# LemonATsu/UNet-PhaseGen

Measured on NVIDIA B200. Metric: audio_seconds_per_second_mag_to_phase_to_wave, higher is better.
Workload: dtype f16x3/f16x2/f16-fp32acc (two-product fp16 on d1,u2; single fp16 product = TF32 operand rounding on u1)

## Files before the change

unet-phasegen_b200/csrc/conv_tc.cu:

```cuda
#include "tc_ptx.cuh"
#include "conv_plan.h"

namespace pg {

struct ConvTcParams {
    ConvPlan plan;
    float* y;
    float4* stats;
    int n_a_slots;
    int b_slot_bytes;
    int n_terms;
    int f16;
    int base_offset_mode;
    int a_mn;
    int epi_mode;
    const float* gamma; const float* beta; float eps;
    ActDst dst0, dst1;
    float2* ss_out;
    const int* clip_rows;
};

constexpr int kThreads = 192;
constexpr int kATileBytes = 128 * 128;
constexpr int kMaxASlots = 8;

struct TileCoord { int co_tile, phase, b0, nt; };

__device__ __forceinline__ int n_bundles(const ConvPlan& p) { return (p.B + p.nb - 1) / p.nb; }
__device__ __forceinline__ int n_co_slabs(const ConvPlan& p) { return p.pair ? p.n_cotiles / 2 : p.n_cotiles; }
__device__ __forceinline__ int tile_OS(const ConvPlan& p) { return p.whole_clip ? 1 : p.OS; }
__device__ __forceinline__ int tile_NT(const ConvPlan& p) { return p.whole_clip ? 1 : p.n_ntiles; }
__device__ __forceinline__ int total_tiles(const ConvPlan& p) { return n_co_slabs(p) * tile_OS(p) * n_bundles(p) * tile_NT(p); }
__device__ __forceinline__ TileCoord decode_tile(const ConvPlan& p, int tile) {
    TileCoord c;
    const int OSx = tile_OS(p), NTx = tile_NT(p);
    const int nbg = n_bundles(p), G = p.clip_group, n_slabs = n_co_slabs(p) * OSx;
    const int tiles_full = n_slabs * G * NTx;
    const int g = tile / tiles_full, r = tile % tiles_full;
    int Gg = nbg - g * G; if (Gg > G) Gg = G;
    const int per_slab = Gg * NTx;
    const int slab = r / per_slab, r2 = r % per_slab;
    c.co_tile = slab / OSx; c.phase = slab % OSx;
    c.b0 = (g * G + r2 / NTx) * p.nb; c.nt = r2 % NTx;
    return c;
}

template <bool PAIR, bool RAGGED>
__global__ void __launch_bounds__(kThreads, 1)
conv_tc_kernel(const __grid_constant__ CUtensorMap map_w_hi, const __grid_constant__ CUtensorMap map_w_lo,
               const __grid_constant__ CUtensorMap map_x_hi, const __grid_constant__ CUtensorMap map_x_lo,
               const __grid_constant__ ConvTcParams prm) {
    extern __shared__ __align__(1024) uint8_t smem_raw[];
    const ConvPlan& pl = prm.plan;
    uint8_t* smem = reinterpret_cast<uint8_t*>((reinterpret_cast<uintptr_t>(smem_raw) + 1023) & ~uintptr_t(1023));
    const int nA = prm.n_a_slots;
    const int bPlane = prm.b_slot_bytes;
    const int a_planes = prm.n_terms == 3 ? 2 : 1;
    const int b_planes = prm.n_terms >= 2 ? 2 : 1;
    uint8_t* a_base = smem;
    uint8_t* b_base = a_base + (size_t)nA * a_planes * kATileBytes;
    uint64_t* bars = reinterpret_cast<uint64_t*>(b_base + 2 * (size_t)b_planes * bPlane);
    uint64_t* fullA = bars;
    uint64_t* emptyA = bars + kMaxASlots;
    uint64_t* fullB = bars + 2 * kMaxASlots;
    uint64_t* emptyB = fullB + 2;
    uint64_t* accFull = emptyB + 2;
    uint64_t* accEmpty = accFull + 2;
    uint32_t* tmem_slot = reinterpret_cast<uint32_t*>(accEmpty + 2);
    uint32_t* epi_tiles = reinterpret_cast<uint32_t*>(reinterpret_cast<uint8_t*>(bars) + 256);

    const int warp = __shfl_sync(0xffffffffu, (int)(threadIdx.x >> 5), 0), lane = threadIdx.x & 31;
    const int n_tiles = total_tiles(pl);
    const bool w_lo = prm.n_terms == 3, x_lo = prm.n_terms >= 2;

    if (warp == 0 && lane == 0) {
        tma_prefetch_desc(&map_w_hi); tma_prefetch_desc(&map_x_hi);
        if (w_lo) tma_prefetch_desc(&map_w_lo);
        if (x_lo) tma_prefetch_desc(&map_x_lo);
        for (int i = 0; i < nA; ++i) { mbar_init(fullA + i, 1); mbar_init(emptyA + i, 1); }
        for (int i = 0; i < 2; ++i) {
            mbar_init(fullB + i, 1); mbar_init(emptyB + i, 1);
            mbar_init(accFull + i, 1); mbar_init(accEmpty + i, PAIR ? 8 : 4);
        }
        fence_barrier_init();
    }
    if (warp == 1) { if (PAIR) tmem_alloc_pair(tmem_slot, 512); else tmem_alloc(tmem_slot, 512); }
    tc_fence_before();
    if (PAIR) cluster_sync_all(); else __syncthreads();
    tc_fence_after();
    const uint32_t tmem_base = __shfl_sync(0xffffffffu, *tmem_slot, 0);
    const int rank = PAIR ? (int)cluster_ctarank() : 0;
    const int tile0 = PAIR ? (int)(blockIdx.x >> 1) : (int)blockIdx.x;
    const int tile_step = PAIR ? (int)(gridDim.x >> 1) : (int)gridDim.x;
    const int half_n = pl.n_tile >> 1;
    const int nb_grp = pl.nb / pl.mgroups;
    const int nb_cta = (PAIR && pl.merged) ? nb_grp >> 1 : nb_grp;
    const int t_phases = pl.whole_clip ? pl.OS : 1;
    const int t_nts = pl.whole_clip ? pl.n_ntiles : 1;
    const int n_sub = pl.merged ? pl.mgroups : t_nts;

    if (warp == 0) {
        {
            uint32_t b_it = 0;
            int a_slot = 0; uint32_t a_ph = 0;
            const uint32_t grp_bytes = (uint32_t)nb_cta * pl.strip_rows * 128u;
            const uint32_t a_bytes = a_planes * kATileBytes;
            const uint32_t b_bytes = b_planes * (uint32_t)bPlane;
            for (int tile = tile0; tile < n_tiles; tile += tile_step) {
                TileCoord tc = decode_tile(pl, tile);
                if (PAIR) tc.co_tile = tc.co_tile * 2 + rank;
                const int m0 = tc.nt * pl.n_tile + ((PAIR && !pl.merged) ? rank * half_n : 0);
                const int clip0 = tc.b0 + ((PAIR && pl.merged) ? rank * nb_cta : 0);
                for (int ch = 0; ch < pl.n_chunks; ++ch) {
                  for (int ph = tc.phase; ph < tc.phase + t_phases; ++ph) {
                    const int ng = pl.n_groups[ph];
                    for (int g = 0; g < ng; ++g) {
                        const ConvGroup grp = pl.groups[ph][g];
                        {
                            const int s = b_it & 1; const uint32_t bph = (b_it >> 1) & 1;
                            mbar_wait(emptyB + s, bph ^ 1);
                            uint8_t* dst = b_base + (size_t)s * b_planes * bPlane;
                            if (elect_one()) {
                                if (PAIR) { if (rank == 0) mbar_expect_tx(fullB + s, 2 * b_bytes); }
                                else mbar_expect_tx(fullB + s, b_bytes);
                                for (int sub = 0; sub < n_sub; ++sub) {
                                    uint8_t* dg = dst + (size_t)sub * grp_bytes;
                                    const int cg = clip0 + (pl.merged ? sub * nb_grp : 0);
                                    const int r0 = m0 + (pl.merged ? 0 : sub * pl.n_tile) + grp.row0;
                                    if (PAIR) {
                                        tma_load_4d_pair(dg, &map_x_hi, fullB + s, ch * 64, grp.parity, r0, cg);
                                        if (x_lo) tma_load_4d_pair(dg + bPlane, &map_x_lo, fullB + s, ch * 64, grp.parity, r0, cg);
                                    } else {
                                        tma_load_4d(dg, &map_x_hi, fullB + s, ch * 64, grp.parity, r0, cg);
                                        if (x_lo) tma_load_4d(dg + bPlane, &map_x_lo, fullB + s, ch * 64, grp.parity, r0, cg);
                                    }
                                }
                            }
                            __syncwarp();
                            ++b_it;
                        }
                        for (int j = 0; j < grp.n_taps; ++j) {
                            const int w_idx = pl.taps[ph][grp.first_tap + j].w_idx;
                            const int s = a_slot; const uint32_t aph = a_ph;
                            mbar_wait(emptyA + s, aph ^ 1);
                            uint8_t* dst = a_base + (size_t)s * a_planes * kATileBytes;
                            if (elect_one()) {
                                if (!PAIR) mbar_expect_tx(fullA + s, a_bytes);
                                else if (rank == 0) mbar_expect_tx(fullA + s, 2 * a_bytes);
                                auto load_w = [&](uint8_t* d, const CUtensorMap* m, int c0, int c1) {
                                    if (PAIR) tma_load_3d_pair(d, m, fullA + s, c0, c1, w_idx);
                                    else tma_load_3d(d, m, fullA + s, c0, c1, w_idx);
                                };
                                if (prm.a_mn) {
                                    for (int h = 0; h < 2; ++h) {
                                        load_w(dst + h * 8192, &map_w_hi, tc.co_tile * 128 + h * 64, ch * 64);
                                        if (w_lo) load_w(dst + kATileBytes + h * 8192, &map_w_lo, tc.co_tile * 128 + h * 64, ch * 64);
                                    }
                                } else {
                                    load_w(dst, &map_w_hi, ch * 64, tc.co_tile * 128);
                                    if (w_lo) load_w(dst + kATileBytes, &map_w_lo, ch * 64, tc.co_tile * 128);
                                }
                            }
                            __syncwarp();
                            if (++a_slot == nA) { a_slot = 0; a_ph ^= 1; }
                        }
                    }
                  }
                }
            }
        }
    } else if (warp == 1) {
        if (rank == 0) {
            uint32_t b_it = 0, t_it = 0;
            int a_slot = 0; uint32_t a_ph = 0;
            const int n_mma = pl.merged ? nb_grp * pl.strip_rows : pl.n_tile;
            const int n_outer = pl.merged ? 1 : t_nts, n_inner = pl.merged ? pl.mgroups : pl.nb;
            const uint32_t dcol_step = pl.merged ? (uint32_t)n_mma : (uint32_t)(pl.n_tile * t_phases * t_nts);
            const uint32_t idesc = (make_idesc_bf16(n_mma, PAIR ? 256 : 128) & ~(prm.f16 ? ((7u << 7) | (7u << 10)) : 0u)) |
                                   (prm.a_mn ? (1u << 15) : 0u);
            const bool a_mn = prm.a_mn != 0;
            auto mma = [&](uint32_t d, uint32_t da, uint32_t db, uint32_t acc_flag) {
                if (elect_one()) { if (PAIR) umma_words_pair(d, da, db, idesc, acc_flag); else umma_words(d, da, db, idesc, acc_flag); }
            };
            const uint32_t a_step = a_mn ? (2048u >> 4) : (32u >> 4);
            auto commit = [&](uint64_t* bar) {
                if (elect_one()) { if (PAIR) umma_commit_pair(bar); else umma_commit(bar); }
                __syncwarp();
            };
            for (int tile = tile0; tile < n_tiles; tile += tile_step, ++t_it) {
                TileCoord tc = decode_tile(pl, tile);
                const int acc = pl.acc_stages == 2 ? (t_it & 1) : 0;
                const uint32_t acc_ph = pl.acc_stages == 2 ? ((t_it >> 1) & 1) : (t_it & 1);
                mbar_wait_sleep(accEmpty + acc, acc_ph ^ 1, 200);
                tc_fence_after();
                const uint32_t d_tmem = tmem_base + acc * 256;
                const uint32_t strip_bytes = (uint32_t)pl.strip_rows * 128u;
                const uint32_t clip_step = (pl.merged ? (uint32_t)nb_cta * strip_bytes : strip_bytes) >> 4;
                for (int ch = 0; ch < pl.n_chunks; ++ch) {
                  for (int ph = tc.phase; ph < tc.phase + t_phases; ++ph) {
                    const int ng = pl.n_groups[ph];
                    const uint32_t dcol_ph = d_tmem + (uint32_t)((ph - tc.phase) * t_nts * pl.n_tile);
                    for (int g = 0; g < ng; ++g) {
                        const ConvGroup grp = pl.groups[ph][g];
                        const int bs = b_it & 1; const uint32_t bph = (b_it >> 1) & 1;
                        mbar_wait(fullB + bs, bph);
                        tc_fence_after();
                        const uint32_t b_hi = smem_u32(b_base + (size_t)bs * b_planes * bPlane);
                        const uint32_t b_lo = b_hi + bPlane;
                        for (int j = 0; j < grp.n_taps; ++j) {
                            const ConvTap tp = pl.taps[ph][grp.first_tap + j];
                            const int as = a_slot; const uint32_t aph = a_ph;
                            mbar_wait(fullA + as, aph);
                            tc_fence_after();
                            const uint32_t a_hi = smem_u32(a_base + (size_t)as * a_planes * kATileBytes);
                            const uint32_t a_lo = a_hi + kATileBytes;
                            const uint32_t sh = (uint32_t)tp.shift * 128u;
                            const uint32_t acc_first = (ch | g | j) ? 1u : 0u;
                            const uint32_t aw_hi = a_mn ? desc_lo_sw128_mn(a_hi, 8192) : desc_lo_sw128(a_hi);
                            const uint32_t aw_lo = a_mn ? desc_lo_sw128_mn(a_lo, 8192) : desc_lo_sw128(a_lo);
                            uint32_t bw_hi = desc_lo_sw128(b_hi + sh), bw_lo = desc_lo_sw128(b_lo + sh);
                            for (int o = 0; o < n_outer; ++o) {
                                uint32_t dcol = dcol_ph + (uint32_t)o * (uint32_t)pl.n_tile;
                                for (int c = 0; c < n_inner; ++c, bw_hi += clip_step, bw_lo += clip_step, dcol += dcol_step) {
                                    if (w_lo) {
#pragma unroll
                                        for (uint32_t kk = 0; kk < 4; ++kk) {
                                            mma(dcol, aw_lo + kk * a_step, bw_hi + kk * 2, kk == 0 ? acc_first : 1u);
                                            mma(dcol, aw_hi + kk * a_step, bw_lo + kk * 2, 1);
                                            mma(dcol, aw_hi + kk * a_step, bw_hi + kk * 2, 1);
                                        }
                                    } else if (x_lo) {
#pragma unroll
                                        for (uint32_t kk = 0; kk < 4; ++kk) {
                                            mma(dcol, aw_hi + kk * a_step, bw_lo + kk * 2, kk == 0 ? acc_first : 1u);
                                            mma(dcol, aw_hi + kk * a_step, bw_hi + kk * 2, 1);
                                        }
                                    } else {
#pragma unroll
                                        for (uint32_t kk = 0; kk < 4; ++kk) mma(dcol, aw_hi + kk * a_step, bw_hi + kk * 2, kk == 0 ? acc_first : 1u);
                                    }
                                }
                            }
                            commit(emptyA + as);
                            if (++a_slot == nA) { a_slot = 0; a_ph ^= 1; }
                        }
                        commit(emptyB + bs);
                        ++b_it;
                    }
                  }
                }
                commit(accFull + acc);
            }
        }
    } else {
        const int q = warp & 3;
        uint32_t* tile = epi_tiles + q * 512;
        uint32_t t_it = 0;
        const int n_parts = t_phases * t_nts;
        const int col_pitch = pl.merged ? pl.strip_rows : pl.n_tile * n_parts;
        bool bad_range = false;
        auto store_f32 = [&](float* base, size_t off0, size_t row_pitch, const float* v, int nv) {
#pragma unroll
            for (int i = 0; i < 16; ++i) tile[i * 32 + lane] = __float_as_uint(v[i]);
            __syncwarp();
#pragma unroll
            for (int t = 0; t < 4; ++t) {
                const int idx = lane + 32 * t, r = idx >> 3, part = idx & 7;
                if (r < nv) {
                    const uint4 w = *reinterpret_cast<const uint4*>(tile + r * 32 + part * 4);
                    *reinterpret_cast<uint4*>(base + off0 + (size_t)r * row_pitch + part * 4) = w;
                }
            }
            __syncwarp();
        };
        auto store_split = [&](const ActDst& d, size_t off0, size_t row_pitch, const float* v, int nv) {
            const int fmt = fmt_of_dtype(d.dtype);
#pragma unroll
            for (int i = 0; i < 16; ++i) {
                const float a = leaky(v[i], d.slope);
                uint16_t h, l;
                split16(a, fmt, h, l);
                if (fmt == PG_FMT_F16 && i < nv) bad_range |= !f16_fits(a);
                tile[i * 32 + lane] = (uint32_t)h | ((uint32_t)l << 16);
            }
            __syncwarp();
            const bool two = d.dtype == PG_DT_BF16_SPLIT || d.dtype == PG_DT_F16_SPLIT;
#pragma unroll
            for (int t = 0; t < 2; ++t) {
                const int idx = lane + 32 * t, r = idx >> 2, part = idx & 3;
                if (r < nv) {
                    const uint4 w0 = *reinterpret_cast<const uint4*>(tile + r * 32 + part * 8);
                    const uint4 w1 = *reinterpret_cast<const uint4*>(tile + r * 32 + part * 8 + 4);
                    uint4 hv, lv;
                    hv.x = __byte_perm(w0.x, w0.y, 0x5410); hv.y = __byte_perm(w0.z, w0.w, 0x5410);
                    hv.z = __byte_perm(w1.x, w1.y, 0x5410); hv.w = __byte_perm(w1.z, w1.w, 0x5410);
                    lv.x = __byte_perm(w0.x, w0.y, 0x7632); lv.y = __byte_perm(w0.z, w0.w, 0x7632);
                    lv.z = __byte_perm(w1.x, w1.y, 0x7632); lv.w = __byte_perm(w1.z, w1.w, 0x7632);
                    const size_t o = off0 + (size_t)r * row_pitch + part * 8;
                    *reinterpret_cast<uint4*>(static_cast<uint16_t*>(d.hi) + o) = hv;
                    if (two) *reinterpret_cast<uint4*>(static_cast<uint16_t*>(d.lo) + o) = lv;
                }
            }
            __syncwarp();
        };
        for (int tile_i = tile0; tile_i < n_tiles; tile_i += tile_step, ++t_it) {
            TileCoord tc = decode_tile(pl, tile_i);
            if (PAIR) tc.co_tile = tc.co_tile * 2 + rank;
            const int acc = pl.acc_stages == 2 ? (t_it & 1) : 0;
            const uint32_t acc_ph = pl.acc_stages == 2 ? ((t_it >> 1) & 1) : (t_it & 1);
            mbar_wait_sleep(accFull + acc, acc_ph, 1000);
            tc_fence_after();
            const int co_base = tc.co_tile * 128 + q * 32;
            const int co = co_base + lane;
            auto part_geom = [&](int p, int L, int& phase, int& m0, int& n_valid) {
                phase = tc.phase + p / t_nts;
                m0 = (tc.nt + p % t_nts) * pl.n_tile;
                const int l_phase = (L - phase + pl.OS - 1) / pl.OS;
                n_valid = l_phase - m0; if (n_valid > pl.n_tile) n_valid = pl.n_tile; if (n_valid < 0) n_valid = 0;
            };
            for (int c = 0; c < pl.nb; ++c) {
                const int b = tc.b0 + c;
                if (b >= pl.B) break;
                const int L_b = RAGGED ? min(__ldg(prm.clip_rows + b), pl.L_out) : pl.L_out;
                const uint32_t tclip = tmem_base + acc * 256 + c * col_pitch + ((uint32_t)(q * 32) << 16);
                if (prm.epi_mode == PG_EPI_RAW) {
                    for (int p = 0; p < n_parts; ++p) {
                        int phase, m0, n_valid;
                        part_geom(p, L_b, phase, m0, n_valid);
                        const uint32_t taddr = tclip + p * pl.n_tile;
                        float sum = 0.f;
                        for (int c0 = 0; c0 < n_valid; c0 += 16) {
                            float v[16];
                            tmem_ld16(taddr + c0, v);
#pragma unroll
                            for (int i = 0; i < 16; ++i) if (c0 + i < n_valid) sum += v[i];
                        }
                        const float mean = n_valid > 0 ? sum / (float)n_valid : 0.f;
                        float m2 = 0.f;
                        const size_t row_pitch = (size_t)pl.OS * pl.out_ld;
                        for (int c0 = 0; c0 < n_valid; c0 += 16) {
                            float v[16];
                            tmem_ld16(taddr + c0, v);
#pragma unroll
                            for (int i = 0; i < 16; ++i) if (c0 + i < n_valid) { const float d = v[i] - mean; m2 += d * d; }
                            const size_t off0 = ((size_t)b * pl.out_rows + (size_t)(m0 + c0) * pl.OS + phase) * pl.out_ld + co_base;
                            store_f32(prm.y, off0, row_pitch, v, n_valid - c0);
                        }
                        if (prm.stats) {
                            const int P = pl.OS * pl.n_ntiles;
                            const int pi = phase * pl.n_ntiles + m0 / pl.n_tile;
                            prm.stats[((size_t)b * P + pi) * pl.C_out + co] = make_float4((float)n_valid, mean, m2, 0.f);
                        }
                    }
                } else {
                    float sc = 1.f, sh = 0.f;
                    if (prm.epi_mode == PG_EPI_NORM_ACT) {
                        float sum = 0.f; int n_tot = 0;
                        for (int p = 0; p < n_parts; ++p) {
                            int phase, m0, n_valid;
                            part_geom(p, L_b, phase, m0, n_valid);
                            n_tot += n_valid;
                            for (int c0 = 0; c0 < n_valid; c0 += 16) {
                                float v[16];
                                tmem_ld16(tclip + p * pl.n_tile + c0, v);
#pragma unroll
                                for (int i = 0; i < 16; ++i) if (c0 + i < n_valid) sum += v[i];
                            }
                        }
                        const float mean = n_tot > 0 ? sum / (float)n_tot : 0.f;
                        float m2 = 0.f;
                        for (int p = 0; p < n_parts; ++p) {
                            int phase, m0, n_valid;
                            part_geom(p, L_b, phase, m0, n_valid);
                            for (int c0 = 0; c0 < n_valid; c0 += 16) {
                                float v[16];
                                tmem_ld16(tclip + p * pl.n_tile + c0, v);
#pragma unroll
                                for (int i = 0; i < 16; ++i) if (c0 + i < n_valid) { const float d = v[i] - mean; m2 += d * d; }
                            }
                        }
                        const float var = n_tot > 0 ? m2 / (float)n_tot : 0.f;
                        sc = (prm.gamma ? __ldg(prm.gamma + co) : 1.f) * rsqrtf(var + prm.eps);
                        sh = (prm.beta ? __ldg(prm.beta + co) : 0.f) - mean * sc;
                        if (prm.ss_out) prm.ss_out[(size_t)b * pl.C_out + co] = make_float2(sc, sh);
                    }
                    for (int p = 0; p < n_parts; ++p) {
// ... 69 lines not shown
}

void device_limits(int* sm_count, int* max_smem) {
    static int sm_dev[kMaxDevices] = {}, smem_dev[kMaxDevices] = {};
    const int slot = current_device_slot();
    if (!sm_dev[slot]) {
        int dev = 0; cudaGetDevice(&dev);
        cudaDeviceGetAttribute(&sm_dev[slot], cudaDevAttrMultiProcessorCount, dev);
        cudaDeviceGetAttribute(&smem_dev[slot], cudaDevAttrMaxSharedMemoryPerBlockOptin, dev);
    }
    *sm_count = sm_dev[slot]; *max_smem = smem_dev[slot];
}

}

extern "C" int pg_conv_epilogue_supported(const pg_conv_desc* d, int mode) {
    using namespace pg;
    PG_REQUIRE(d, "pg_conv_epilogue_supported: null descriptor");
    if (mode == PG_EPI_RAW) return 1;
    if (mode != PG_EPI_ACT && mode != PG_EPI_NORM_ACT) return 0;
    if (d->precision == PG_PREC_FP32_SIMT || d->C_in % 64 || d->C_out % 128) return 0;
    if (mode == PG_EPI_ACT) return 1;
    pg_conv_desc dd = *d;
    dd.tc_whole_clip = 1;
    ConvPlan pl;
    if (conv_plan_build(&dd, &pl) != PG_OK) return 0;
    return (pl.whole_clip || (pl.OS == 1 && pl.n_ntiles == 1)) ? 1 : 0;
}

static int conv_tc_launch(const pg_conv_desc* d, const uint16_t* x_hi, const uint16_t* x_lo, const uint16_t* w_hi,
                          const uint16_t* w_lo, float* y, float* stats, const pg_conv_epilogue* epi, const int* out_rows,
                          pg_stream stream) {
    using namespace pg;
    const int epi_mode = epi ? epi->mode : PG_EPI_RAW;
    PG_REQUIRE(d && x_hi && w_hi && (y || epi_mode != PG_EPI_RAW), "pg_conv_tc: null pointer");
    PG_REQUIRE(epi_mode == PG_EPI_RAW || epi_mode == PG_EPI_ACT || epi_mode == PG_EPI_NORM_ACT, "pg_conv_tc: bad epilogue mode %d", epi_mode);
    PG_REQUIRE(d->precision >= PG_PREC_BF16X3 && d->precision <= PG_PREC_F16, "pg_conv_tc: precision must be BF16X3, BF16, F16X3, F16X2 or F16");
    const int n_terms = (d->precision == PG_PREC_BF16X3 || d->precision == PG_PREC_F16X3) ? 3 : d->precision == PG_PREC_F16X2 ? 2 : 1;
    const bool three = n_terms == 3;
    PG_REQUIRE(n_terms < 3 || w_lo, "pg_conv_tc: weight lo plane required for the three-product precisions");
    PG_REQUIRE(n_terms < 2 || x_lo, "pg_conv_tc: activation lo plane required for this precision");
    PG_REQUIRE(d->C_in % 64 == 0 && d->C_out % 128 == 0, "pg_conv_tc: needs C_in %% 64 == 0 and C_out %% 128 == 0 (got %d, %d)", d->C_in, d->C_out);
    PG_REQUIRE(d->in_ld % 8 == 0, "pg_conv_tc: input row pitch must be a multiple of 8 elements");
    PG_REQUIRE(d->tc_base_offset_mode == 0, "pg_conv_tc: descriptor base-offset mode 0 is the only supported one (the UMMA swizzle is a "
               "function of the absolute shared-memory address: profiles/r01_tc_probe.log)");
    ConvTcParams prm;
    pg_conv_desc d_local = *d;
    if (const char* e = getenv("PG_TC_PAIR")) d_local.tc_cta_pair = atoi(e);
    d_local.tc_whole_clip = epi_mode == PG_EPI_NORM_ACT ? 1 : 0;
    d = &d_local;
    int rc = conv_plan_build(d, &prm.plan);
    if (rc != PG_OK) return rc;
    const ConvPlan& pl = prm.plan;
    prm.epi_mode = epi_mode; prm.gamma = nullptr; prm.beta = nullptr; prm.eps = 1e-5f; prm.ss_out = nullptr;
    prm.clip_rows = out_rows;
    const bool ragged = out_rows != nullptr;
    if ((rc = to_act_dst(nullptr, 0, &prm.dst0, "pg_conv_tc", "dst0")) != PG_OK) return rc;
    prm.dst1 = prm.dst0;
    if (epi_mode != PG_EPI_RAW) {
        PG_REQUIRE(epi_mode != PG_EPI_NORM_ACT || pl.whole_clip || (pl.OS == 1 && pl.n_ntiles == 1),
                   "pg_conv_tc: the fused per-clip norm needs a whole clip per tile (L_out %d does not fit 512 accumulator columns)", pl.L_out);
        if ((rc = to_act_dst(&epi->dst0, d->C_out, &prm.dst0, "pg_conv_tc", "dst0")) != PG_OK) return rc;
        if ((rc = to_act_dst(&epi->dst1, d->C_out, &prm.dst1, "pg_conv_tc", "dst1")) != PG_OK) return rc;
        PG_REQUIRE(prm.dst0.dtype || prm.dst1.dtype, "pg_conv_tc: fused epilogue without a destination");
        for (const ActDst* a : {&prm.dst0, &prm.dst1})
            PG_REQUIRE(!a->dtype || (a->ld % 8 == 0 && a->ch_off % 8 == 0 && a->batch_stride % 8 == 0 && (reinterpret_cast<uintptr_t>(a->hi) & 15) == 0 &&
                                      (reinterpret_cast<uintptr_t>(a->lo) & 15) == 0),
                       "pg_conv_tc: fused-epilogue destinations need 16-byte aligned planes and ld, ch_off, batch_stride multiples of 8");
        prm.gamma = epi->gamma; prm.beta = epi->beta; prm.eps = epi->eps; prm.ss_out = reinterpret_cast<float2*>(epi->scale_shift);
    } else {
        PG_REQUIRE(d->out_ld % 4 == 0 && (reinterpret_cast<uintptr_t>(y) & 15) == 0, "pg_conv_tc: y must be 16-byte aligned with out_ld a multiple of 4");
    }
    int g_sm_count, g_max_smem;
    device_limits(&g_sm_count, &g_max_smem);
    prm.y = y; prm.stats = reinterpret_cast<float4*>(stats);
    prm.n_terms = n_terms;
    prm.f16 = (d->precision == PG_PREC_F16X3 || d->precision == PG_PREC_F16X2 || d->precision == PG_PREC_F16) ? 1 : 0;
    prm.base_offset_mode = d->tc_base_offset_mode;
    prm.a_mn = d->weights_mn_major ? 1 : 0;
    const int nb_grp = pl.nb / pl.mgroups;
    const int nb_cta = (pl.pair && pl.merged) ? nb_grp / 2 : nb_grp;
    prm.b_slot_bytes = (pl.merged ? pl.mgroups : (pl.whole_clip ? pl.n_ntiles : 1)) * nb_cta * pl.strip_rows * 128;
    const int a_planes = n_terms == 3 ? 2 : 1, b_planes = n_terms >= 2 ? 2 : 1;
    const int fixed = 2 * b_planes * prm.b_slot_bytes + 1024  + 256  + 8192  +
                      (pl.merged ? 2048 : 0);
    int nA = (g_max_smem - fixed) / (a_planes * kATileBytes);
    if (nA > kMaxASlots) nA = kMaxASlots;
    PG_REQUIRE(nA >= 2, "pg_conv_tc: strip of %d rows leaves no room for the weight ring", pl.strip_rows);
    prm.n_a_slots = nA;
    const size_t smem_bytes = (size_t)fixed + (size_t)nA * a_planes * kATileBytes;

    CUtensorMap mw_hi, mw_lo, mx_hi, mx_lo;
    {
        const uint64_t inner = prm.a_mn ? d->C_out : d->C_in, outer = prm.a_mn ? d->C_in : d->C_out;
        uint64_t dims[3] = {inner, outer, (uint64_t)d->k};
        uint64_t str[2] = {inner * 2, inner * outer * 2};
        uint32_t box[3] = {64, prm.a_mn ? 64u : 128u, 1};
        if ((rc = encode_bf16_map(&mw_hi, w_hi, 3, dims, str, box, "w_hi")) != PG_OK) return rc;
        if ((rc = encode_bf16_map(&mw_lo, three ? w_lo : w_hi, 3, dims, str, box, "w_lo")) != PG_OK) return rc;
    }
    {
        const int IS = pl.IS;
        uint64_t dims[4] = {(uint64_t)d->C_in, (uint64_t)IS, (uint64_t)((d->L_in + IS - 1) / IS), (uint64_t)d->B};
        uint64_t str[3] = {(uint64_t)d->in_ld * 2, (uint64_t)d->in_ld * 2 * IS, (uint64_t)d->in_rows * d->in_ld * 2};
        uint32_t box[4] = {64, 1, (uint32_t)pl.strip_rows, (uint32_t)nb_cta};
        PG_REQUIRE(d->in_rows >= ((d->L_in + IS - 1) / IS) * IS, "pg_conv_tc: in_rows %d too small for L_in %d at stride %d", d->in_rows, d->L_in, IS);
        if ((rc = encode_bf16_map(&mx_hi, x_hi, 4, dims, str, box, "x_hi")) != PG_OK) return rc;
        if ((rc = encode_bf16_map(&mx_lo, n_terms >= 2 ? x_lo : x_hi, 4, dims, str, box, "x_lo")) != PG_OK) return rc;
    }
    const bool pair = pl.pair != 0;
    auto kernel = pair ? (ragged ? conv_tc_kernel<true, true> : conv_tc_kernel<true, false>)
                       : (ragged ? conv_tc_kernel<false, true> : conv_tc_kernel<false, false>);
    {
        static size_t configured_dev[kMaxDevices][4] = {};
        const int variant = 2 * pair + ragged;
        size_t* configured = configured_dev[current_device_slot()];
        if (smem_bytes > configured[variant]) {
            cudaError_t e = cudaFuncSetAttribute(kernel, cudaFuncAttributeMaxDynamicSharedMemorySize, (int)smem_bytes);
            if (e != cudaSuccess) { set_error("conv_tc: cannot opt in to %zu bytes of shared memory: %s", smem_bytes, cudaGetErrorString(e)); return PG_ERR_CUDA; }
            configured[variant] = smem_bytes;
        }
    }
    {
        const int nbg = (pl.B + pl.nb - 1) / pl.nb;
        const double bundle_bytes = (double)pl.nb * d->in_rows * d->in_ld * (n_terms >= 2 ? 4.0 : 2.0);
        int G = (int)(64.0e6 / bundle_bytes);
        if (const char* e = getenv("PG_TC_CLIP_GROUP")) G = atoi(e);
        if (G < 1) G = 1;
        if (G > nbg) G = nbg;
        prm.plan.clip_group = G;
    }
    const int n_tiles = (pair ? pl.n_cotiles / 2 : pl.n_cotiles) * ((pl.B + pl.nb - 1) / pl.nb) * (pl.whole_clip ? 1 : pl.OS * pl.n_ntiles);
    int units = pair ? g_sm_count / 2 : g_sm_count;
    if (const char* e = getenv("PG_TC_MAX_CTAS")) {
        const int cap = atoi(e);
        if (cap > 0 && units > (pair ? cap / 2 : cap)) units = pair ? cap / 2 : cap;
    }
    if (d->tc_max_ctas > 0 && units > (pair ? (d->tc_max_ctas + 1) / 2 : d->tc_max_ctas)) units = pair ? (d->tc_max_ctas + 1) / 2 : d->tc_max_ctas;
    if (units > n_tiles) units = n_tiles;
    cudaLaunchConfig_t cfg = {};
    cfg.gridDim = dim3(pair ? 2 * units : units);
    cfg.blockDim = dim3(kThreads);
    cfg.dynamicSmemBytes = smem_bytes;
    cfg.stream = reinterpret_cast<cudaStream_t>(stream);
    cudaLaunchAttribute attr[1];
    attr[0].id = cudaLaunchAttributeClusterDimension;
    attr[0].val.clusterDim.x = pair ? 2 : 1; attr[0].val.clusterDim.y = 1; attr[0].val.clusterDim.z = 1;
    cfg.attrs = attr; cfg.numAttrs = 1;
    cudaError_t le = cudaLaunchKernelEx(&cfg, kernel, mw_hi, mw_lo, mx_hi, mx_lo, prm);
    if (le != cudaSuccess) { set_error("conv_tc_kernel launch failed: %s", cudaGetErrorString(le)); return PG_ERR_CUDA; }
    return check_launch("conv_tc_kernel");
}

extern "C" int pg_conv_tc(const pg_conv_desc* d, const uint16_t* x_hi, const uint16_t* x_lo, const uint16_t* w_hi,
                          const uint16_t* w_lo, float* y, float* stats, const pg_conv_epilogue* epi, pg_stream stream) {
    return conv_tc_launch(d, x_hi, x_lo, w_hi, w_lo, y, stats, epi, nullptr, stream);
}

extern "C" int pg_conv_tc_ragged(const pg_conv_desc* d, const uint16_t* x_hi, const uint16_t* x_lo, const uint16_t* w_hi,
                                 const uint16_t* w_lo, float* y, float* stats, const pg_conv_epilogue* epi, const int* out_rows,
                                 pg_stream stream) {
    PG_REQUIRE(out_rows, "pg_conv_tc_ragged: null per-clip row table");
    return conv_tc_launch(d, x_hi, x_lo, w_hi, w_lo, y, stats, epi, out_rows, stream);
}
```

unet-phasegen_b200/csrc/tc_ptx.cuh:

```cuda
#pragma once
#include <cuda.h>

#include <cstdio>
#include <cstdlib>

#include "common.cuh"

namespace pg {

__device__ __forceinline__ uint32_t smem_u32(const void* p) { return (uint32_t)__cvta_generic_to_shared(p); }

__device__ __forceinline__ void mbar_init(uint64_t* bar, uint32_t count) {
    asm volatile("mbarrier.init.shared::cta.b64 [%0], %1;" ::"r"(smem_u32(bar)), "r"(count));
}
__device__ __forceinline__ void mbar_expect_tx(uint64_t* bar, uint32_t bytes) {
    asm volatile("mbarrier.arrive.expect_tx.shared::cta.b64 _, [%0], %1;" ::"r"(smem_u32(bar)), "r"(bytes) : "memory");
}
__device__ __forceinline__ void mbar_arrive(uint64_t* bar) {
    asm volatile("mbarrier.arrive.shared::cta.b64 _, [%0];" ::"r"(smem_u32(bar)) : "memory");
}
__device__ __forceinline__ bool mbar_try_wait(uint64_t* bar, uint32_t parity) {
    uint32_t ok;
    asm volatile(
        "{\n\t.reg .pred p;\n\t"
        "mbarrier.try_wait.parity.shared::cta.b64 p, [%1], %2;\n\t"
        "selp.u32 %0, 1, 0, p;\n\t}"
        : "=r"(ok) : "r"(smem_u32(bar)), "r"(parity) : "memory");
    return ok != 0;
}
__device__ __forceinline__ void mbar_wait(uint64_t* bar, uint32_t parity) {
    if (mbar_try_wait(bar, parity)) return;
    const long long t0 = clock64();
    for (uint32_t spins = 1; !mbar_try_wait(bar, parity); ++spins) {
        if ((spins & 1023u) == 0 && clock64() - t0 > 4000000000ll) {
            printf("phasegen conv_tc: mbarrier timeout (block %d thread %d bar %u parity %u)\n",
                   (int)blockIdx.x, (int)threadIdx.x, smem_u32(bar), parity);
            __trap();
        }
    }
}
__device__ __forceinline__ void mbar_wait_sleep(uint64_t* bar, uint32_t parity, unsigned ns) {
    if (mbar_try_wait(bar, parity)) return;
    const long long t0 = clock64();
    for (uint32_t spins = 1; !mbar_try_wait(bar, parity); ++spins) {
        __nanosleep(ns);
        if ((spins & 255u) == 0 && clock64() - t0 > 4000000000ll) {
            printf("phasegen conv_tc: mbarrier timeout (block %d thread %d bar %u parity %u)\n",
                   (int)blockIdx.x, (int)threadIdx.x, smem_u32(bar), parity);
            __trap();
        }
    }
}
__device__ __forceinline__ bool elect_one() {
    uint32_t pred;
    asm volatile("{\n\t.reg .pred p;\n\telect.sync _|p, 0xffffffff;\n\tselp.u32 %0, 1, 0, p;\n\t}" : "=r"(pred));
    return pred != 0;
}
__device__ __forceinline__ void fence_barrier_init() { asm volatile("fence.mbarrier_init.release.cluster;" ::: "memory"); }
__device__ __forceinline__ void fence_proxy_async() { asm volatile("fence.proxy.async.shared::cta;" ::: "memory"); }
__device__ __forceinline__ void tc_fence_before() { asm volatile("tcgen05.fence::before_thread_sync;" ::: "memory"); }
__device__ __forceinline__ void tc_fence_after() { asm volatile("tcgen05.fence::after_thread_sync;" ::: "memory"); }

__device__ __forceinline__ void tma_load_3d(void* dst, const CUtensorMap* map, uint64_t* bar, int c0, int c1, int c2) {
    asm volatile(
        "cp.async.bulk.tensor.3d.shared::cluster.global.tile.mbarrier::complete_tx::bytes [%0], [%1, {%3, %4, %5}], [%2];"
        ::"r"(smem_u32(dst)), "l"(map), "r"(smem_u32(bar)), "r"(c0), "r"(c1), "r"(c2) : "memory");
}
__device__ __forceinline__ void tma_load_4d(void* dst, const CUtensorMap* map, uint64_t* bar, int c0, int c1, int c2, int c3) {
    asm volatile(
        "cp.async.bulk.tensor.4d.shared::cluster.global.tile.mbarrier::complete_tx::bytes [%0], [%1, {%3, %4, %5, %6}], [%2];"
        ::"r"(smem_u32(dst)), "l"(map), "r"(smem_u32(bar)), "r"(c0), "r"(c1), "r"(c2), "r"(c3) : "memory");
}
__device__ __forceinline__ void tma_prefetch_desc(const CUtensorMap* map) {
    asm volatile("prefetch.tensormap [%0];" ::"l"(map) : "memory");
}

__device__ __forceinline__ void tmem_alloc(uint32_t* dst_smem, uint32_t cols) {
    asm volatile("tcgen05.alloc.cta_group::1.sync.aligned.shared::cta.b32 [%0], %1;" ::"r"(smem_u32(dst_smem)), "r"(cols) : "memory");
    asm volatile("tcgen05.relinquish_alloc_permit.cta_group::1.sync.aligned;" ::: "memory");
}
__device__ __forceinline__ void tmem_dealloc(uint32_t addr, uint32_t cols) {
    asm volatile("tcgen05.dealloc.cta_group::1.sync.aligned.b32 %0, %1;" ::"r"(addr), "r"(cols) : "memory");
}
__device__ __forceinline__ void umma_bf16(uint32_t d_tmem, uint64_t a_desc, uint64_t b_desc, uint32_t idesc, uint32_t accumulate) {
    asm volatile(
        "{\n\t.reg .pred p;\n\t"
        "setp.ne.b32 p, %4, 0;\n\t"
        "tcgen05.mma.cta_group::1.kind::f16 [%0], %1, %2, %3, p;\n\t}"
        ::"r"(d_tmem), "l"(a_desc), "l"(b_desc), "r"(idesc), "r"(accumulate) : "memory");
}
__device__ __forceinline__ void umma_commit(uint64_t* bar) {
    asm volatile("tcgen05.commit.cta_group::1.mbarrier::arrive::one.shared::cluster.b64 [%0];" ::"r"(smem_u32(bar)) : "memory");
}
__device__ __forceinline__ void tmem_ld16(uint32_t taddr, float* v) {
    uint32_t r[16];
    asm volatile(
        "tcgen05.ld.sync.aligned.32x32b.x16.b32 {%0,%1,%2,%3,%4,%5,%6,%7,%8,%9,%10,%11,%12,%13,%14,%15}, [%16];"
        : "=r"(r[0]), "=r"(r[1]), "=r"(r[2]), "=r"(r[3]), "=r"(r[4]), "=r"(r[5]), "=r"(r[6]), "=r"(r[7]),
          "=r"(r[8]), "=r"(r[9]), "=r"(r[10]), "=r"(r[11]), "=r"(r[12]), "=r"(r[13]), "=r"(r[14]), "=r"(r[15])
        : "r"(taddr));
    asm volatile("tcgen05.wait::ld.sync.aligned;" ::: "memory");
#pragma unroll
    for (int i = 0; i < 16; ++i) v[i] = __uint_as_float(r[i]);
}

constexpr uint32_t kPeerBitMask = 0xFEFFFFFFu;

__device__ __forceinline__ uint32_t cluster_ctarank() { uint32_t r; asm volatile("mov.u32 %0, %%cluster_ctarank;" : "=r"(r)); return r; }
__device__ __forceinline__ void cluster_sync_all() {
    asm volatile("barrier.cluster.arrive.release.aligned;" ::: "memory");
    asm volatile("barrier.cluster.wait.acquire.aligned;" ::: "memory");
}
__device__ __forceinline__ void tma_load_3d_pair(void* dst, const CUtensorMap* map, uint64_t* bar, int c0, int c1, int c2) {
    asm volatile(
        "cp.async.bulk.tensor.3d.cta_group::2.shared::cluster.global.mbarrier::complete_tx::bytes [%0], [%1, {%3, %4, %5}], [%2];"
        ::"r"(smem_u32(dst)), "l"(map), "r"(smem_u32(bar) & kPeerBitMask), "r"(c0), "r"(c1), "r"(c2) : "memory");
}
__device__ __forceinline__ void tma_load_4d_pair(void* dst, const CUtensorMap* map, uint64_t* bar, int c0, int c1, int c2, int c3) {
    asm volatile(
        "cp.async.bulk.tensor.4d.cta_group::2.shared::cluster.global.mbarrier::complete_tx::bytes [%0], [%1, {%3, %4, %5, %6}], [%2];"
        ::"r"(smem_u32(dst)), "l"(map), "r"(smem_u32(bar) & kPeerBitMask), "r"(c0), "r"(c1), "r"(c2), "r"(c3) : "memory");
}
__device__ __forceinline__ void tmem_alloc_pair(uint32_t* dst_smem, uint32_t cols) {
    asm volatile("tcgen05.alloc.cta_group::2.sync.aligned.shared::cta.b32 [%0], %1;" ::"r"(smem_u32(dst_smem)), "r"(cols) : "memory");
    asm volatile("tcgen05.relinquish_alloc_permit.cta_group::2.sync.aligned;" ::: "memory");
}
__device__ __forceinline__ void tmem_dealloc_pair(uint32_t addr, uint32_t cols) {
    asm volatile("tcgen05.dealloc.cta_group::2.sync.aligned.b32 %0, %1;" ::"r"(addr), "r"(cols) : "memory");
}
__device__ __forceinline__ void umma_bf16_pair(uint32_t d_tmem, uint64_t a_desc, uint64_t b_desc, uint32_t idesc, uint32_t accumulate) {
    asm volatile(
        "{\n\t.reg .pred p;\n\t"
        "setp.ne.b32 p, %4, 0;\n\t"
        "tcgen05.mma.cta_group::2.kind::f16 [%0], %1, %2, %3, p;\n\t}"
        ::"r"(d_tmem), "l"(a_desc), "l"(b_desc), "r"(idesc), "r"(accumulate) : "memory");
}
__device__ __forceinline__ void umma_commit_pair(uint64_t* bar) {
    asm volatile("tcgen05.commit.cta_group::2.mbarrier::arrive::one.shared::cluster.multicast::cluster.b64 [%0], %1;"
                 ::"r"(smem_u32(bar)), "h"((uint16_t)3) : "memory");
}
__device__ __forceinline__ void mbar_arrive_leader(uint64_t* bar) {
    asm volatile("mbarrier.arrive.release.cluster.shared::cluster.b64 _, [%0];" ::"r"(smem_u32(bar) & kPeerBitMask) : "memory");
}

__device__ __forceinline__ uint64_t make_desc_sw128(uint32_t saddr, int base_offset_mode) {
    uint64_t d = 0;
    d |= (uint64_t)((saddr & 0x3FFFF) >> 4);
    d |= (uint64_t)0 << 16;
    d |= (uint64_t)(1024 >> 4) << 32;
    d |= (uint64_t)1 << 46;
    if (base_offset_mode) d |= (uint64_t)((saddr >> 7) & 7) << 49;
    d |= (uint64_t)2 << 61;
    return d;
}
constexpr uint32_t kDescHiSw128 = (1024u >> 4) | (1u << 14) | (2u << 29);
__device__ __forceinline__ uint32_t desc_lo_sw128(uint32_t saddr) { return (saddr & 0x3FFFF) >> 4; }
__device__ __forceinline__ uint32_t desc_lo_sw128_mn(uint32_t saddr, uint32_t lbo_bytes) {
    return ((saddr & 0x3FFFF) >> 4) | (((lbo_bytes >> 4) & 0x3FFF) << 16);
}
__device__ __forceinline__ void umma_words(uint32_t d_tmem, uint32_t a_lo, uint32_t b_lo, uint32_t idesc, uint32_t accumulate) {
    asm volatile(
        "{\n\t.reg .pred p;\n\t.reg .b64 da, db;\n\t"
        "setp.ne.b32 p, %4, 0;\n\t"
        "mov.b64 da, {%1, %5};\n\t"
        "mov.b64 db, {%2, %5};\n\t"
        "tcgen05.mma.cta_group::1.kind::f16 [%0], da, db, %3, p;\n\t}"
        ::"r"(d_tmem), "r"(a_lo), "r"(b_lo), "r"(idesc), "r"(accumulate), "r"(kDescHiSw128) : "memory");
}
__device__ __forceinline__ void umma_words_pair(uint32_t d_tmem, uint32_t a_lo, uint32_t b_lo, uint32_t idesc, uint32_t accumulate) {
    asm volatile(
        "{\n\t.reg .pred p;\n\t.reg .b64 da, db;\n\t"
        "setp.ne.b32 p, %4, 0;\n\t"
        "mov.b64 da, {%1, %5};\n\t"
        "mov.b64 db, {%2, %5};\n\t"
        "tcgen05.mma.cta_group::2.kind::f16 [%0], da, db, %3, p;\n\t}"
        ::"r"(d_tmem), "r"(a_lo), "r"(b_lo), "r"(idesc), "r"(accumulate), "r"(kDescHiSw128) : "memory");
}

__device__ __forceinline__ uint32_t make_idesc_bf16(int n, int m = 128) {
    return (1u << 4) | (1u << 7) | (1u << 10) | ((uint32_t)(n >> 3) << 17) | ((uint32_t)(m >> 4) << 24);
}


__device__ __forceinline__ uint64_t make_desc_sw128_mn(uint32_t saddr, uint32_t lbo_bytes) {
    uint64_t d = 0;
    d |= (uint64_t)((saddr & 0x3FFFF) >> 4);
    d |= (uint64_t)((lbo_bytes >> 4) & 0x3FFF) << 16;
// ... 19 lines not shown
```

Before: 46240.

## Add register-resident epilogue variant with 8 epilogue warps and setmaxnreg rebalancing

Adds a REG kernel variant with 384 threads, selected when there is a single accumulator stage, two output units and n_tile fits in 176 columns. Eight epilogue warps each drain a whole accumulator column block from TMEM into registers with batched non-blocking loads, then release the accumulator early. Norm statistics are exchanged between the two warp halves through small smem buffers guarded by mbarriers. setmaxnreg moves registers from the control warps to the epilogue warps. The aim is to shorten the epilogue's critical path and free TMEM sooner, at the cost of heavy register pressure, possible spills from the shift_down loop, and a more complex cross-warp handshake.

```diff
diff --git a/unet-phasegen_b200/csrc/conv_tc.cu b/unet-phasegen_b200/csrc/conv_tc.cu
--- a/unet-phasegen_b200/csrc/conv_tc.cu
+++ b/unet-phasegen_b200/csrc/conv_tc.cu
@@ -45,8 +45,68 @@
     return c;
 }
 
-template <bool PAIR, bool RAGGED>
-__global__ void __launch_bounds__(kThreads, 1)
+template <int ROWS = 16>
+__device__ __forceinline__ void epi_store_f32(uint32_t* tile, int lane, float* base, size_t off0, size_t row_pitch,
+                                              const float* v, int nv) {
+#pragma unroll
+    for (int i = 0; i < ROWS; ++i) tile[i * 32 + lane] = __float_as_uint(v[i]);
+    __syncwarp();
+#pragma unroll
+    for (int t = 0; t < ROWS / 4; ++t) {
+        const int idx = lane + 32 * t, r = idx >> 3, part = idx & 7;
+        if (r < nv) {
+            const uint4 w = *reinterpret_cast<const uint4*>(tile + r * 32 + part * 4);
+            *reinterpret_cast<uint4*>(base + off0 + (size_t)r * row_pitch + part * 4) = w;
+        }
+    }
+    __syncwarp();
+}
+template <int ROWS = 16>
+__device__ __forceinline__ void epi_store_split(uint32_t* tile, int lane, const ActDst& d, size_t off0, size_t row_pitch,
+                                                const float* v, int nv, bool& bad_range) {
+    const int fmt = fmt_of_dtype(d.dtype);
+#pragma unroll
+    for (int i = 0; i < ROWS; ++i) {
+        const float a = leaky(v[i], d.slope);
+        uint16_t h, l;
+        split16(a, fmt, h, l);
+        if (fmt == PG_FMT_F16 && i < nv) bad_range |= !f16_fits(a);
+        tile[i * 32 + lane] = (uint32_t)h | ((uint32_t)l << 16);
+    }
+    __syncwarp();
+    const bool two = d.dtype == PG_DT_BF16_SPLIT || d.dtype == PG_DT_F16_SPLIT;
+#pragma unroll
+    for (int t = 0; t < ROWS / 8; ++t) {
+        const int idx = lane + 32 * t, r = idx >> 2, part = idx & 3;
+        if (r < nv) {
+            const uint4 w0 = *reinterpret_cast<const uint4*>(tile + r * 32 + part * 8);
+            const uint4 w1 = *reinterpret_cast<const uint4*>(tile + r * 32 + part * 8 + 4);
+            uint4 hv, lv;
+            hv.x = __byte_perm(w0.x, w0.y, 0x5410); hv.y = __byte_perm(w0.z, w0.w, 0x5410);
+            hv.z = __byte_perm(w1.x, w1.y, 0x5410); hv.w = __byte_perm(w1.z, w1.w, 0x5410);
+            lv.x = __byte_perm(w0.x, w0.y, 0x7632); lv.y = __byte_perm(w0.z, w0.w, 0x7632);
+            lv.z = __byte_perm(w1.x, w1.y, 0x7632); lv.w = __byte_perm(w1.z, w1.w, 0x7632);
+            const size_t o = off0 + (size_t)r * row_pitch + part * 8;
+            *reinterpret_cast<uint4*>(static_cast<uint16_t*>(d.hi) + o) = hv;
+            if (two) *reinterpret_cast<uint4*>(static_cast<uint16_t*>(d.lo) + o) = lv;
+        }
+    }
+    __syncwarp();
+}
+
+constexpr int kThreadsReg = 384;
+constexpr int kRegCols = 176;
+constexpr uint32_t kRegCtl = 56, kRegEpi = 224;
+__device__ __forceinline__ void shift_down16(float* v) {
+#pragma unroll
+    for (int i = 0; i < kRegCols - 16; ++i) v[i] = v[i + 16];
+}
+__host__ __device__ constexpr int conv_threads(bool reg) { return reg ? kThreadsReg : kThreads; }
+__host__ __device__ constexpr int epi_bar_bytes(bool reg) { return reg ? 512 : 256; }
+__host__ __device__ constexpr int epi_smem_bytes(bool reg) { return reg ? 8 * 1024 + 4 * 64 * 4 : 4 * 2048; }
+
+template <bool PAIR, bool RAGGED, bool REG>
+__global__ void __launch_bounds__(conv_threads(REG), 1)
 conv_tc_kernel(const __grid_constant__ CUtensorMap map_w_hi, const __grid_constant__ CUtensorMap map_w_lo,
                const __grid_constant__ CUtensorMap map_x_hi, const __grid_constant__ CUtensorMap map_x_lo,
                const __grid_constant__ ConvTcParams prm) {
@@ -67,7 +127,9 @@
     uint64_t* accFull = emptyB + 2;
     uint64_t* accEmpty = accFull + 2;
     uint32_t* tmem_slot = reinterpret_cast<uint32_t*>(accEmpty + 2);
-    uint32_t* epi_tiles = reinterpret_cast<uint32_t*>(reinterpret_cast<uint8_t*>(bars) + 256);
+    uint64_t* xfer = bars + 32;
+    uint32_t* epi_tiles = reinterpret_cast<uint32_t*>(reinterpret_cast<uint8_t*>(bars) + epi_bar_bytes(REG));
+    float* xfer_val = reinterpret_cast<float*>(epi_tiles + 8 * 256);
 
     const int warp = __shfl_sync(0xffffffffu, (int)(threadIdx.x >> 5), 0), lane = threadIdx.x & 31;
     const int n_tiles = total_tiles(pl);
@@ -80,8 +142,9 @@
         for (int i = 0; i < nA; ++i) { mbar_init(fullA + i, 1); mbar_init(emptyA + i, 1); }
         for (int i = 0; i < 2; ++i) {
             mbar_init(fullB + i, 1); mbar_init(emptyB + i, 1);
-            mbar_init(accFull + i, 1); mbar_init(accEmpty + i, PAIR ? 8 : 4);
-        }
+            mbar_init(accFull + i, 1); mbar_init(accEmpty + i, (PAIR ? 2 : 1) * (REG ? 8 : 4));
+        }
+        if (REG) for (int i = 0; i < 8; ++i) mbar_init(xfer + i, 32);
         fence_barrier_init();
     }
     if (warp == 1) { if (PAIR) tmem_alloc_pair(tmem_slot, 512); else tmem_alloc(tmem_slot, 512); }
@@ -98,6 +161,7 @@
     const int t_phases = pl.whole_clip ? pl.OS : 1;
     const int t_nts = pl.whole_clip ? pl.n_ntiles : 1;
     const int n_sub = pl.merged ? pl.mgroups : t_nts;
+    if (REG && warp < 4) setmaxnreg_dec<kRegCtl>();
 
     if (warp == 0) {
         {
@@ -252,6 +316,141 @@
                 commit(accFull + acc);
             }
         }
+    } else if (REG) {
+        if (warp >= 4) {
+            setmaxnreg_inc<kRegEpi>();
+            const int q = warp & 3, h = (warp >> 2) - 1;
+            uint32_t* tile = epi_tiles + (warp - 4) * 256;
+            float* xv = xfer_val + q * 64;
+            uint64_t* to_h1 = xfer + q;
+            uint64_t* to_h0 = xfer + 4 + q;
+            uint32_t t_it = 0;
+            const int n_parts = t_phases * t_nts;
+            const int c = h / n_parts, p = h % n_parts;
+            const bool hand_over = prm.epi_mode == PG_EPI_NORM_ACT && n_parts == 2;
+            bool bad_range = false;
+            for (int tile_i = tile0; tile_i < n_tiles; tile_i += tile_step, ++t_it) {
+                TileCoord tc = decode_tile(pl, tile_i);
+                if (PAIR) tc.co_tile = tc.co_tile * 2 + rank;
+                mbar_wait_sleep(accFull, t_it & 1, 200);
+                tc_fence_after();
+                uint32_t r[kRegCols];
+                const uint32_t taddr = tmem_base + (uint32_t)(h * pl.n_tile) + ((uint32_t)(q * 32) << 16);
+#pragma unroll
+                for (int k = 0; k < kRegCols / 16; ++k) tmem_ld16_nowait(taddr + k * 16, r + k * 16);
+                tmem_ld_wait();
+                tc_fence_before();
+                __syncwarp();
+                if (lane == 0) { if (PAIR) mbar_arrive_leader(accEmpty); else mbar_arrive(accEmpty); }
+                float v[kRegCols];
+#pragma unroll
+                for (int i = 0; i < kRegCols; ++i) v[i] = __uint_as_float(r[i]);
+
+                const int b = tc.b0 + c;
+                if (b >= pl.B) continue;
+                const int L_b = RAGGED ? min(__ldg(prm.clip_rows + b), pl.L_out) : pl.L_out;
+                const int co_base = tc.co_tile * 128 + q * 32;
+                const int co = co_base + lane;
+                auto part_geom = [&](int pp, int L, int& phase, int& m0, int& n_valid) {
+                    phase = tc.phase + pp / t_nts;
+                    m0 = (tc.nt + pp % t_nts) * pl.n_tile;
+                    const int l_phase = (L - phase + pl.OS - 1) / pl.OS;
+                    n_valid = l_phase - m0; if (n_valid > pl.n_tile) n_valid = pl.n_tile; if (n_valid < 0) n_valid = 0;
+                };
+                if (prm.epi_mode == PG_EPI_RAW) {
+                    int phase, m0, n_valid;
+                    part_geom(p, L_b, phase, m0, n_valid);
+                    float sum = 0.f;
+#pragma unroll
+                    for (int i = 0; i < kRegCols; ++i) if (i < n_valid) sum += v[i];
+                    const float mean = n_valid > 0 ? sum / (float)n_valid : 0.f;
+                    float m2 = 0.f;
+                    const size_t row_pitch = (size_t)pl.OS * pl.out_ld;
+#pragma unroll 1
+                    for (int c0 = 0; c0 < n_valid; c0 += 16) {
+#pragma unroll
+                        for (int i = 0; i < 16; ++i) if (c0 + i < n_valid) { const float d = v[i] - mean; m2 += d * d; }
+                        const size_t off0 = ((size_t)b * pl.out_rows + (size_t)(m0 + c0) * pl.OS + phase) * pl.out_ld + co_base;
+                        epi_store_f32<8>(tile, lane, prm.y, off0, row_pitch, v, n_valid - c0);
+                        if (n_valid - c0 > 8) epi_store_f32<8>(tile, lane, prm.y, off0 + 8 * row_pitch, row_pitch, v + 8, n_valid - c0 - 8);
+                        shift_down16(v);
+                    }
+                    if (prm.stats) {
+                        const int P = pl.OS * pl.n_ntiles;
+                        const int pi = phase * pl.n_ntiles + m0 / pl.n_tile;
+                        prm.stats[((size_t)b * P + pi) * pl.C_out + co] = make_float4((float)n_valid, mean, m2, 0.f);
+                    }
+                } else {
+                    float sc = 1.f, sh = 0.f;
+                    if (prm.epi_mode == PG_EPI_NORM_ACT) {
+                        int n_tot = 0, n_mine = 0;
+                        for (int pp = 0; pp < n_parts; ++pp) {
+                            int phase, m0, n_valid;
+                            part_geom(pp, L_b, phase, m0, n_valid);
+                            n_tot += n_valid;
+                            if (pp == p) n_mine = n_valid;
+                        }
+                        float sum = 0.f;
+                        if (hand_over && h == 1) { mbar_wait_sleep(to_h1, 0, 20); sum = xv[lane]; }
+#pragma unroll
+                        for (int i = 0; i < kRegCols; ++i) if (i < n_mine) sum += v[i];
+                        if (hand_over) {
+                            if (h == 0) { xv[lane] = sum; mbar_arrive(to_h1); mbar_wait_sleep(to_h0, 0, 20); sum = xv[32 + lane]; }
+                            else { xv[32 + lane] = sum; mbar_arrive(to_h0); }
+                        }
+                        const float mean = n_tot > 0 ? sum / (float)n_tot : 0.f;
+                        float m2 = 0.f;
+                        if (hand_over && h == 1) { mbar_wait_sleep(to_h1, 1, 20); m2 = xv[lane]; }
+#pragma unroll
+                        for (int i = 0; i < kRegCols; ++i) if (i < n_mine) { const float d = v[i] - mean; m2 += d * d; }
+                        if (hand_over) {
+                            if (h == 0) { xv[lane] = m2; mbar_arrive(to_h1); mbar_wait_sleep(to_h0, 1, 20); m2 = xv[32 + lane]; }
+                            else { xv[32 + lane] = m2; mbar_arrive(to_h0); }
+                        }
+                        const float var = n_tot > 0 ? m2 / (float)n_tot : 0.f;
+                        sc = (prm.gamma ? __ldg(prm.gamma + co) : 1.f) * rsqrtf(var + prm.eps);
+                        sh = (prm.beta ? __ldg(prm.beta + co) : 0.f) - mean * sc;
+                        if (prm.ss_out && p == 0) prm.ss_out[(size_t)b * pl.C_out + co] = make_float2(sc, sh);
+                    }
+                    int phase, m0, n_valid, n_own = 0;
+                    part_geom(p, pl.L_out, phase, m0, n_valid);
+                    if (RAGGED) { int ph_, m0_; part_geom(p, L_b, ph_, m0_, n_own); }
+#pragma unroll 1
+                    for (int c0 = 0; c0 < n_valid; c0 += 16) {
+                        float* vc = v;
+#pragma unroll
+                        for (int i = 0; i < 16; ++i) vc[i] = fmaf(vc[i], sc, sh);
+                        if (RAGGED) {
+#pragma unroll
+                            for (int i = 0; i < 16; ++i) if (c0 + i >= n_own) vc[i] = 0.f;
+                        }
+                        const size_t row0 = (size_t)(m0 + c0) * pl.OS + phase;
+#pragma unroll
+                        for (int k = 0; k < 2; ++k) {
+                            const ActDst& d = k ? prm.dst1 : prm.dst0;
+                            if (!d.dtype) continue;
+                            const size_t off0 = (size_t)b * d.batch_stride + row0 * d.ld + d.ch_off + co_base;
+                            const size_t rp = (size_t)pl.OS * d.ld;
+                            if (d.dtype == PG_DT_F32) {
+                                float a[16];
+#pragma unroll
+                                for (int i = 0; i < 16; ++i) a[i] = leaky(vc[i], d.slope);
+                                epi_store_f32<8>(tile, lane, static_cast<float*>(d.hi), off0, rp, a, n_valid - c0);
+                                if (n_valid - c0 > 8) epi_store_f32<8>(tile, lane, static_cast<float*>(d.hi), off0 + 8 * rp, rp, a + 8, n_valid - c0 - 8);
+                            } else {
+                                epi_store_split<8>(tile, lane, d, off0, rp, vc, n_valid - c0, bad_range);
+                                if (n_valid - c0 > 8) epi_store_split<8>(tile, lane, d, off0 + 8 * rp, rp, vc + 8, n_valid - c0 - 8, bad_range);
+                            }
+                        }
+                        shift_down16(v);
+                    }
+                }
+            }
+            if (bad_range) {
+                if (prm.dst0.range_flag) atomicOr(prm.dst0.range_flag, 1);
+                else if (prm.dst1.range_flag) atomicOr(prm.dst1.range_flag, 1);
+            }
+        }
     } else {
         const int q = warp & 3;
         uint32_t* tile = epi_tiles + q * 512;
@@ -260,48 +459,10 @@
         const int col_pitch = pl.merged ? pl.strip_rows : pl.n_tile * n_parts;
         bool bad_range = false;
         auto store_f32 = [&](float* base, size_t off0, size_t row_pitch, const float* v, int nv) {
-#pragma unroll
-            for (int i = 0; i < 16; ++i) tile[i * 32 + lane] = __float_as_uint(v[i]);
-            __syncwarp();
-#pragma unroll
-            for (int t = 0; t < 4; ++t) {
-                const int idx = lane + 32 * t, r = idx >> 3, part = idx & 7;
-                if (r < nv) {
-                    const uint4 w = *reinterpret_cast<const uint4*>(tile + r * 32 + part * 4);
-                    *reinterpret_cast<uint4*>(base + off0 + (size_t)r * row_pitch + part * 4) = w;
-                }
-            }
-            __syncwarp();
+            epi_store_f32(tile, lane, base, off0, row_pitch, v, nv);
         };
         auto store_split = [&](const ActDst& d, size_t off0, size_t row_pitch, const float* v, int nv) {
-            const int fmt = fmt_of_dtype(d.dtype);
-#pragma unroll
-            for (int i = 0; i < 16; ++i) {
-                const float a = leaky(v[i], d.slope);
-                uint16_t h, l;
-                split16(a, fmt, h, l);
-                if (fmt == PG_FMT_F16 && i < nv) bad_range |= !f16_fits(a);
-                tile[i * 32 + lane] = (uint32_t)h | ((uint32_t)l << 16);
-            }
-            __syncwarp();
-            const bool two = d.dtype == PG_DT_BF16_SPLIT || d.dtype == PG_DT_F16_SPLIT;
-#pragma unroll
-            for (int t = 0; t < 2; ++t) {
-                const int idx = lane + 32 * t, r = idx >> 2, part = idx & 3;
-                if (r < nv) {
-                    const uint4 w0 = *reinterpret_cast<const uint4*>(tile + r * 32 + part * 8);
-                    const uint4 w1 = *reinterpret_cast<const uint4*>(tile + r * 32 + part * 8 + 4);
-                    uint4 hv, lv;
-                    hv.x = __byte_perm(w0.x, w0.y, 0x5410); hv.y = __byte_perm(w0.z, w0.w, 0x5410);
-                    hv.z = __byte_perm(w1.x, w1.y, 0x5410); hv.w = __byte_perm(w1.z, w1.w, 0x5410);
-                    lv.x = __byte_perm(w0.x, w0.y, 0x7632); lv.y = __byte_perm(w0.z, w0.w, 0x7632);
-                    lv.z = __byte_perm(w1.x, w1.y, 0x7632); lv.w = __byte_perm(w1.z, w1.w, 0x7632);
-                    const size_t o = off0 + (size_t)r * row_pitch + part * 8;
-                    *reinterpret_cast<uint4*>(static_cast<uint16_t*>(d.hi) + o) = hv;
-                    if (two) *reinterpret_cast<uint4*>(static_cast<uint16_t*>(d.lo) + o) = lv;
-                }
-            }
-            __syncwarp();
+            epi_store_split(tile, lane, d, off0, row_pitch, v, nv, bad_range);
         };
         for (int tile_i = tile0; tile_i < n_tiles; tile_i += tile_step, ++t_it) {
             TileCoord tc = decode_tile(pl, tile_i);
@@ -537,8 +698,10 @@
     const int nb_cta = (pl.pair && pl.merged) ? nb_grp / 2 : nb_grp;
     prm.b_slot_bytes = (pl.merged ? pl.mgroups : (pl.whole_clip ? pl.n_ntiles : 1)) * nb_cta * pl.strip_rows * 128;
     const int a_planes = n_terms == 3 ? 2 : 1, b_planes = n_terms >= 2 ? 2 : 1;
-    const int fixed = 2 * b_planes * prm.b_slot_bytes + 1024  + 256  + 8192  +
-                      (pl.merged ? 2048 : 0);
+    const int n_units = pl.merged ? 0 : pl.nb * (pl.whole_clip ? pl.OS * pl.n_ntiles : 1);
+    const bool reg = pl.acc_stages == 1 && n_units == 2 && pl.n_tile <= kRegCols;
+    const int fixed = 2 * b_planes * prm.b_slot_bytes + 1024  + epi_bar_bytes(reg)  +
+                      epi_smem_bytes(reg)  + (pl.merged ? 2048 : 0);
     int nA = (g_max_smem - fixed) / (a_planes * kATileBytes);
     if (nA > kMaxASlots) nA = kMaxASlots;
     PG_REQUIRE(nA >= 2, "pg_conv_tc: strip of %d rows leaves no room for the weight ring", pl.strip_rows);
@@ -564,11 +727,13 @@
         if ((rc = encode_bf16_map(&mx_lo, n_terms >= 2 ? x_lo : x_hi, 4, dims, str, box, "x_lo")) != PG_OK) return rc;
     }
     const bool pair = pl.pair != 0;
-    auto kernel = pair ? (ragged ? conv_tc_kernel<true, true> : conv_tc_kernel<true, false>)
-                       : (ragged ? conv_tc_kernel<false, true> : conv_tc_kernel<false, false>);
+    auto kernel = reg ? (pair ? (ragged ? conv_tc_kernel<true, true, true> : conv_tc_kernel<true, false, true>)
+                              : (ragged ? conv_tc_kernel<false, true, true> : conv_tc_kernel<false, false, true>))
+                      : (pair ? (ragged ? conv_tc_kernel<true, true, false> : conv_tc_kernel<true, false, false>)
+                              : (ragged ? conv_tc_kernel<false, true, false> : conv_tc_kernel<false, false, false>));
     {
-        static size_t configured_dev[kMaxDevices][4] = {};
-        const int variant = 2 * pair + ragged;
+        static size_t configured_dev[kMaxDevices][8] = {};
+        const int variant = 4 * reg + 2 * pair + ragged;
         size_t* configured = configured_dev[current_device_slot()];
         if (smem_bytes > configured[variant]) {
             cudaError_t e = cudaFuncSetAttribute(kernel, cudaFuncAttributeMaxDynamicSharedMemorySize, (int)smem_bytes);
@@ -595,7 +760,7 @@
     if (units > n_tiles) units = n_tiles;
     cudaLaunchConfig_t cfg = {};
     cfg.gridDim = dim3(pair ? 2 * units : units);
-    cfg.blockDim = dim3(kThreads);
+    cfg.blockDim = dim3(conv_threads(reg));
     cfg.dynamicSmemBytes = smem_bytes;
     cfg.stream = reinterpret_cast<cudaStream_t>(stream);
     cudaLaunchAttribute attr[1];
diff --git a/unet-phasegen_b200/csrc/tc_ptx.cuh b/unet-phasegen_b200/csrc/tc_ptx.cuh
--- a/unet-phasegen_b200/csrc/tc_ptx.cuh
+++ b/unet-phasegen_b200/csrc/tc_ptx.cuh
@@ -103,6 +103,17 @@
 #pragma unroll
     for (int i = 0; i < 16; ++i) v[i] = __uint_as_float(r[i]);
 }
+__device__ __forceinline__ void tmem_ld16_nowait(uint32_t taddr, uint32_t* r) {
+    asm volatile(
+        "tcgen05.ld.sync.aligned.32x32b.x16.b32 {%0,%1,%2,%3,%4,%5,%6,%7,%8,%9,%10,%11,%12,%13,%14,%15}, [%16];"
+        : "=r"(r[0]), "=r"(r[1]), "=r"(r[2]), "=r"(r[3]), "=r"(r[4]), "=r"(r[5]), "=r"(r[6]), "=r"(r[7]),
+          "=r"(r[8]), "=r"(r[9]), "=r"(r[10]), "=r"(r[11]), "=r"(r[12]), "=r"(r[13]), "=r"(r[14]), "=r"(r[15])
+        : "r"(taddr));
+}
+__device__ __forceinline__ void tmem_ld_wait() { asm volatile("tcgen05.wait::ld.sync.aligned;" ::: "memory"); }
+
+template <uint32_t N> __device__ __forceinline__ void setmaxnreg_dec() { asm volatile("setmaxnreg.dec.sync.aligned.u32 %0;" ::"n"(N)); }
+template <uint32_t N> __device__ __forceinline__ void setmaxnreg_inc() { asm volatile("setmaxnreg.inc.sync.aligned.u32 %0;" ::"n"(N)); }
 
 constexpr uint32_t kPeerBitMask = 0xFEFFFFFFu;
 
```

New measurement: 47020, median of 6. 1.02x the previous value.
